# tl32rodan/DCVC

Measured on AMD Instinct MI355X. Metric: encode+decode fps @1920x1080 per GPU; bpp bit-exact + PSNR Δ<1e-4 dB vs ref, higher is better.
Workload: dtype f32 (convs on split-fp16 f16x3 MFMA, fp32 accumulation); 1 GPU; C3 DCVC-DC RGB 1920x1080 (pad 1920x1088) IP=32 write mode; gop=32, precision=split, q_index=0, stream_part=8, parallelism=sequence-sharded x1, 3 GOP lane(s) per GPU, lanes=3, step=one frame on each of 3 lane(s)

## Files before the change

### dcvc_amd/csrc/hip/sdc.hip

```cpp
#include "common.h"
#include "split.h"

namespace {

constexpr int kNW = 8, kNT = kNW * 64;
constexpr int TH = 8, TW = 16;
constexpr int HW_ = TW + 2, NPH = (TH + 2) * HW_;
constexpr int HR = 192;

struct DP {
  const float *x;
  int H, W, xcs, xco;
  float *y;
  int ycs, yco;
  const uint16_t *w;
  int wbytes;
  const float *b1, *wdw, *bdw, *b2, *ba;
  float slope;
  int tiles_x, ntiles;
  int *ovf;
};

template <int CIN, int COUT, bool ADAPT>
struct DG {
  static constexpr int KCI = (CIN + 31) / 32;
  static constexpr int NTI = (CIN + 15) / 16, NTO = (COUT + 15) / 16;
  static constexpr int CI16 = NTI * 16, CO16 = NTO * 16;
  static constexpr int W1 = KCI * CI16 * 32, W2 = KCI * CO16 * 32, WA = ADAPT ? KCI * CO16 * 32 : 0;
  static constexpr int NWH = 2 * (W1 + W2 + WA);
  static constexpr int XI = KCI * HR * 32;
  static constexpr int DI = KCI * TH * TW * 32;
  static constexpr size_t OX = 0, OD = OX + (size_t)2 * XI * 2, OW = OD + (size_t)2 * DI * 2;
  static constexpr size_t OC = OW + (size_t)NWH * 2;
  static constexpr int NC = CIN * 11 + 2 * COUT;
  static constexpr size_t LDS = OC + (size_t)NC * 4;
  static constexpr int QP = CIN / 8;
  static constexpr int PP = (NPH * QP + kNT - 1) / kNT;
};

__device__ __forceinline__ float lrelu(float v, float s) { return fmaxf(v, v * s); }

template <int CIN, int COUT, bool ADAPT>
__global__ void __launch_bounds__(kNT) sdc_kernel(DP p) {
  SplitRange rg(p.ovf);
  typedef DG<CIN, COUT, ADAPT> G_;
  constexpr int KCI = G_::KCI, NTI = G_::NTI, NTO = G_::NTO, CO16 = G_::CO16, CI16 = G_::CI16;
  constexpr int XI = G_::XI, DI = G_::DI, QP = G_::QP, PP = G_::PP;
  extern __shared__ __align__(16) unsigned char smem[];
  uint16_t *Xh = reinterpret_cast<uint16_t *>(smem + G_::OX), *Xl = Xh + XI;
  uint16_t *Dh = reinterpret_cast<uint16_t *>(smem + G_::OD), *Dl = Dh + DI;
  uint16_t *W1h = reinterpret_cast<uint16_t *>(smem + G_::OW), *W1l = W1h + G_::W1;
  uint16_t *W2h = W1l + G_::W1, *W2l = W2h + G_::W2;
  uint16_t *WAh = W2l + G_::W2, *WAl = WAh + G_::WA;
  float *Lb1 = reinterpret_cast<float *>(smem + G_::OC), *Lbdw = Lb1 + CIN, *Lwdw = Lbdw + CIN;
  float *Lb2 = Lwdw + 9 * CIN, *Lba = Lb2 + COUT;
  auto t1p = [&](int r, int c) -> float * {
    return reinterpret_cast<float *>((c & 16) ? Xl : Xh) + (((c >> 5) * HR + r) * 16 + (c & 15));
  };

  const int tid = threadIdx.x;
  const int wave = tid >> 6, lane = tid & 63;
  const int col = lane & 15, hi = lane >> 4;
  const int G = gridDim.x;
  int g = blockIdx.x;
  if ((G & 7) == 0) g = (g & 7) * (G >> 3) + (g >> 3);
  if (g >= p.ntiles) return;

  {
    const __amdgpu_buffer_rsrc_t wr =
        __builtin_amdgcn_make_buffer_rsrc(const_cast<uint16_t *>(p.w), (short)0, p.wbytes, 0x00020000);
    constexpr int ND = G_::NWH * 2 / 1024;
    for (int i = wave; i < ND; i += kNW)
      __builtin_amdgcn_raw_ptr_buffer_load_lds(wr, (__attribute__((address_space(3))) void *)(W1h + i * 512), 16,
                                               i * 1024 + lane * 16, 0, 0, 0);
    for (int i = tid; i < G_::NC; i += kNT) {
      float v;
      if (i < CIN) v = p.b1[i];
      else if (i < 2 * CIN) v = p.bdw[i - CIN];
      else if (i < 11 * CIN) v = p.wdw[i - 2 * CIN];
      else if (i < 11 * CIN + COUT) v = p.b2[i - 11 * CIN];
      else v = ADAPT ? p.ba[i - 11 * CIN - COUT] : 0.f;
      Lb1[i] = v;
    }
  }

  const __amdgpu_buffer_rsrc_t xr = __builtin_amdgcn_make_buffer_rsrc(
      const_cast<float *>(p.x), (short)0,
      (int)((int64_t)p.H * p.W * p.xcs * 4 < 0x7fff0000 ? (int64_t)p.H * p.W * p.xcs * 4 : 0x7fff0000), 0x00020000);
  int pyx[PP], prel[PP], pofs[PP];
#pragma unroll
  for (int u = 0; u < PP; ++u) {
    const int it = tid + u * kNT;
    pyx[u] = -1;
    prel[u] = 0;
    pofs[u] = 0;
    if (it < NPH * QP) {
      const int pix = it / QP, q = it - pix * QP;
      const int hy = pix / HW_, hx = pix - hy * HW_;
      pyx[u] = (hy << 8) | hx;
      prel[u] = ((hy - 1) * p.W + (hx - 1)) * p.xcs + p.xco + q * 8;
      pofs[u] = swz((q >> 2) * HR + pix, q & 3);
    }
  }
  float pf[PP][8];
  auto prefetch = [&](int t) {
    const int oy0 = (t / p.tiles_x) * TH, ox0 = (t % p.tiles_x) * TW;
    const int base = oy0 * p.W + ox0;
#pragma unroll
    for (int u = 0; u < PP; ++u) {
      const int gy = oy0 - 1 + (pyx[u] >> 8), gx = ox0 - 1 + (pyx[u] & 255);
      const bool in = pyx[u] >= 0 && (unsigned)gy < (unsigned)p.H && (unsigned)gx < (unsigned)p.W;
      const int o = in ? (base * p.xcs + prel[u]) * 4 : 0x7fffffe0;
      const f32x4 a = __builtin_bit_cast(f32x4, __builtin_amdgcn_raw_buffer_load_b128(xr, o, 0, 0));
      const f32x4 b = __builtin_bit_cast(f32x4, __builtin_amdgcn_raw_buffer_load_b128(xr, o + 16, 0, 0));
#pragma unroll
      for (int j = 0; j < 4; ++j) {
        pf[u][j] = a[j];
        pf[u][4 + j] = b[j];
      }
    }
  };
  prefetch(g);

  auto zero_pad = [&]() {
    if constexpr (CIN % 32 != 0) {
      constexpr int PADQ = KCI * 4 - QP;
      for (int it = tid; it < HR * PADQ; it += kNT) {
        const int row = it / PADQ, q = QP + it % PADQ;
        const int o = swz((q >> 2) * HR + row, q & 3);
        *reinterpret_cast<u32x4_t *>(Xh + o) = u32x4_t{0u, 0u, 0u, 0u};
        *reinterpret_cast<u32x4_t *>(Xl + o) = u32x4_t{0u, 0u, 0u, 0u};
      }
    }
  };

  wait_vm_lgkm();
  for (int t = g; t < p.ntiles; t += G) {
    const int oy0 = (t / p.tiles_x) * TH, ox0 = (t % p.tiles_x) * TW;
    raw_barrier();
#pragma unroll
    for (int u = 0; u < PP; ++u) {
      u32x4_t h, l;
      rg.add8(pf[u]);
      split8(pf[u], h, l);
      if (pyx[u] >= 0) {
        *reinterpret_cast<u32x4_t *>(Xh + pofs[u]) = h;
        *reinterpret_cast<u32x4_t *>(Xl + pofs[u]) = l;
      }
    }
    zero_pad();
    wait_lgkm();
    raw_barrier();
    if (t + G < p.ntiles) prefetch(t + G);

    f32x4 idn[NTO];
    if constexpr (ADAPT) {
      f32x4 am[NTO], ac[NTO];
#pragma unroll
      for (int j = 0; j < NTO; ++j) {
        am[j] = f32x4{0.f, 0.f, 0.f, 0.f};
        ac[j] = f32x4{0.f, 0.f, 0.f, 0.f};
      }
      const int hr = (wave + 1) * HW_ + 1 + col;
#pragma unroll
      for (int kc = 0; kc < KCI; ++kc) {
        const int ob = swz(kc * HR + hr, hi);
        const f16x8 bh = *reinterpret_cast<const f16x8 *>(Xh + ob), bl = *reinterpret_cast<const f16x8 *>(Xl + ob);
#pragma unroll
        for (int j = 0; j < NTO; ++j) {
          const int oa = swz(kc * CO16 + j * 16 + col, hi);
          const f16x8 ah = *reinterpret_cast<const f16x8 *>(WAh + oa), al = *reinterpret_cast<const f16x8 *>(WAl + oa);
          am[j] = __builtin_amdgcn_mfma_f32_16x16x32_f16(ah, bh, am[j], 0, 0, 0);
          ac[j] = __builtin_amdgcn_mfma_f32_16x16x32_f16(ah, bl, ac[j], 0, 0, 0);
          ac[j] = __builtin_amdgcn_mfma_f32_16x16x32_f16(al, bh, ac[j], 0, 0, 0);
        }
      }
#pragma unroll
      for (int j = 0; j < NTO; ++j) {
        const int n = j * 16 + hi * 4;
#pragma unroll
        for (int e = 0; e < 4; ++e) idn[j][e] = (am[j][e] + ac[j][e] * kLoInv) + Lba[n + e < COUT ? n + e : 0];
      }
      wait_lgkm();
      raw_barrier();
    }

    for (int ht = wave; ht < HR / 16; ht += kNW) {
      f32x4 tm[NTI], tc[NTI];
#pragma unroll
      for (int j = 0; j < NTI; ++j) {
        tm[j] = f32x4{0.f, 0.f, 0.f, 0.f};
        tc[j] = f32x4{0.f, 0.f, 0.f, 0.f};
      }
      const int r = ht * 16 + col;
#pragma unroll
      for (int kc = 0; kc < KCI; ++kc) {
        const int ob = swz(kc * HR + r, hi);
        const f16x8 bh = *reinterpret_cast<const f16x8 *>(Xh + ob), bl = *reinterpret_cast<const f16x8 *>(Xl + ob);
#pragma unroll
        for (int j = 0; j < NTI; ++j) {
          const int oa = swz(kc * CI16 + j * 16 + col, hi);
          const f16x8 ah = *reinterpret_cast<const f16x8 *>(W1h + oa), al = *reinterpret_cast<const f16x8 *>(W1l + oa);
          tm[j] = __builtin_amdgcn_mfma_f32_16x16x32_f16(ah, bh, tm[j], 0, 0, 0);
          tc[j] = __builtin_amdgcn_mfma_f32_16x16x32_f16(ah, bl, tc[j], 0, 0, 0);
          tc[j] = __builtin_amdgcn_mfma_f32_16x16x32_f16(al, bh, tc[j], 0, 0, 0);
        }
      }
      const int hy = r / HW_, hx = r - hy * HW_;
      const int gy = oy0 - 1 + hy, gx = ox0 - 1 + hx;
      const bool inside = r < NPH && (unsigned)gy < (unsigned)p.H && (unsigned)gx < (unsigned)p.W;
      wave_lds_sync();
#pragma unroll
      for (int j = 0; j < NTI; ++j) {
        const int n = j * 16 + hi * 4;
        if (n >= CIN) continue;
        f32x4 v;
#pragma unroll
        for (int e = 0; e < 4; ++e) v[e] = inside ? lrelu((tm[j][e] + tc[j][e] * kLoInv) + Lb1[n + e], p.slope) : 0.f;
        *reinterpret_cast<f32x4 *>(t1p(r, n)) = v;
      }
    }
    wait_lgkm();
    raw_barrier();

    {
      constexpr int CG = CIN / 4;
      constexpr int R = kNT / (CG * TW) >= 4 ? 4 : kNT / (CG * TW) >= 2 ? 2 : 1;
      constexpr int RR = TH / R;
      static_assert(CG * TW * R <= kNT && TH % R == 0, "P2 tasks");
      if (tid < CG * TW * R) {
        const int cg = tid % CG, rest = tid / CG;
        const int ix = rest % TW, y0 = (rest / TW) * RR;
        const int c = cg * 4;
        f32x4 wv[9];
#pragma unroll
        for (int k = 0; k < 9; ++k) wv[k] = *reinterpret_cast<const f32x4 *>(Lwdw + k * CIN + c);
        const float4 bd = *reinterpret_cast<const float4 *>(Lbdw + c);
        f32x4 win[3][3];
#pragma unroll
        for (int r = 0; r < 2; ++r)
#pragma unroll
          for (int dx = 0; dx < 3; ++dx)
            win[r][dx] = *reinterpret_cast<const f32x4 *>(t1p((y0 + r) * HW_ + ix + dx, c));
#pragma unroll
        for (int i = 0; i < RR; ++i) {
#pragma unroll
          for (int dx = 0; dx < 3; ++dx)
            win[(i + 2) % 3][dx] = *reinterpret_cast<const f32x4 *>(t1p((y0 + i + 2) * HW_ + ix + dx, c));
          f32x4 a = f32x4{0.f, 0.f, 0.f, 0.f};
#pragma unroll
          for (int dy = 0; dy < 3; ++dy)
#pragma unroll
            for (int dx = 0; dx < 3; ++dx)
#pragma unroll
              for (int e = 0; e < 4; ++e) a[e] = __builtin_fmaf(wv[dy * 3 + dx][e], win[(i + dy) % 3][dx][e], a[e]);
          float v[4];
          v[0] = a[0] + bd.x;
          v[1] = a[1] + bd.y;
          v[2] = a[2] + bd.z;
          v[3] = a[3] + bd.w;
          rg.add4(v);
          const auto h01 = __builtin_amdgcn_cvt_pkrtz(v[0], v[1]);
          const auto h23 = __builtin_amdgcn_cvt_pkrtz(v[2], v[3]);
          const uint32_t l01 = pk(split_lo(v[0], (float)h01[0]), split_lo(v[1], (float)h01[1]));
          const uint32_t l23 = pk(split_lo(v[2], (float)h23[0]), split_lo(v[3], (float)h23[1]));
          const int px = (y0 + i) * TW + ix;
          const int o = swz((c >> 5) * (TH * TW) + px, (c & 31) >> 3) + (c & 7);
          typedef unsigned int u32x2_t __attribute__((ext_vector_type(2)));
          *reinterpret_cast<u32x2_t *>(Dh + o) = u32x2_t{__builtin_bit_cast(uint32_t, h01), __builtin_bit_cast(uint32_t, h23)};
          *reinterpret_cast<u32x2_t *>(Dl + o) = u32x2_t{l01, l23};
        }
      }
      if constexpr (CIN % 32 != 0) {
        constexpr int PADQ = KCI * 4 - CIN / 8;
        for (int it = tid; it < TH * TW * PADQ; it += kNT) {
          const int px = it / PADQ, q = CIN / 8 + it % PADQ;
          const int o = swz((q >> 2) * (TH * TW) + px, q & 3);
          *reinterpret_cast<u32x4_t *>(Dh + o) = u32x4_t{0u, 0u, 0u, 0u};
          *reinterpret_cast<u32x4_t *>(Dl + o) = u32x4_t{0u, 0u, 0u, 0u};
        }
      }
    }
    wait_lgkm();
    raw_barrier();

    {
      f32x4 cm[NTO], cc[NTO];
#pragma unroll
      for (int j = 0; j < NTO; ++j) {
        cm[j] = f32x4{0.f, 0.f, 0.f, 0.f};
        cc[j] = f32x4{0.f, 0.f, 0.f, 0.f};
      }
#pragma unroll
      for (int kc = 0; kc < KCI; ++kc) {
        const int ob = swz(kc * (TH * TW) + wave * TW + col, hi);
        const f16x8 bh = *reinterpret_cast<const f16x8 *>(Dh + ob), bl = *reinterpret_cast<const f16x8 *>(Dl + ob);
#pragma unroll
        for (int j = 0; j < NTO; ++j) {
          const int oa = swz(kc * CO16 + j * 16 + col, hi);
          const f16x8 ah = *reinterpret_cast<const f16x8 *>(W2h + oa), al = *reinterpret_cast<const f16x8 *>(W2l + oa);
          cm[j] = __builtin_amdgcn_mfma_f32_16x16x32_f16(ah, bh, cm[j], 0, 0, 0);
          cc[j] = __builtin_amdgcn_mfma_f32_16x16x32_f16(ah, bl, cc[j], 0, 0, 0);
          cc[j] = __builtin_amdgcn_mfma_f32_16x16x32_f16(al, bh, cc[j], 0, 0, 0);
        }
      }
      const int gy = oy0 + wave, gx = ox0 + col;
      if (gy < p.H && gx < p.W) {
        const int64_t pix = (int64_t)gy * p.W + gx;
#pragma unroll
        for (int j = 0; j < NTO; ++j) {
          const int n = j * 16 + hi * 4;
          if (n >= COUT) continue;
          f32x4 id;
          if constexpr (ADAPT) id = idn[j];
          else id = *reinterpret_cast<const f32x4 *>(p.x + pix * p.xcs + p.xco + n);
          f32x4 v;
#pragma unroll
          for (int e = 0; e < 4; ++e) v[e] = ((cm[j][e] + cc[j][e] * kLoInv) + Lb2[n + e]) + id[e];
          *reinterpret_cast<f32x4 *>(p.y + pix * p.ycs + p.yco + n) = v;
        }
      }
    }
  }
  wait_vm_lgkm();
}

int g_cus = 0;

template <int CIN, int COUT, bool ADAPT>
int run(DP p, hipStream_t st) {
  typedef DG<CIN, COUT, ADAPT> G_;
  static_assert(G_::LDS <= 160 * 1024, "LDS");
  static_assert(G_::NWH * 2 % 1024 == 0, "weight images in whole 1-KiB pieces");
  p.tiles_x = (p.W + TW - 1) / TW;
  const int64_t nt = (int64_t)p.tiles_x * ((p.H + TH - 1) / TH);
  if (nt <= 0) return DCVC_HIP_OK;
  p.ntiles = (int)nt;
  if (g_cus <= 0) {
    int dev = 0;
    hipDeviceProp_t prop;
    if (hipGetDevice(&dev) != hipSuccess || hipGetDeviceProperties(&prop, dev) != hipSuccess) return DCVC_HIP_ELAUNCH;
    g_cus = prop.multiProcessorCount;
  }
  int G = g_cus;
  if (G > p.ntiles) G = p.ntiles;
  auto kern = sdc_kernel<CIN, COUT, ADAPT>;
  dcvc_note_kernel("sdc_kernel<%d, %d, %s>@%lld", CIN, COUT, bname(ADAPT), (long long)G * kNT);
  dcvc_ensure_lds(reinterpret_cast<const void *>(kern), (int)G_::LDS);
  hipLaunchKernelGGL(kern, dim3((unsigned)G), dim3(kNT), G_::LDS, st, p);
  DCVC_LAUNCH_CHECK();
  return DCVC_HIP_OK;
}

bool supported(int cin, int cout, bool adapt) {
  return (cin == 64 && cout == 48 && adapt) || (cin == 48 && cout == 32 && adapt) ||
         (cin == 64 && cout == 64 && !adapt) || (cin == 32 && cout == 64 && adapt) ||
         (cin == 48 && cout == 48 && !adapt) || (cin == 32 && cout == 32 && !adapt);
}

}

extern "C" int64_t dcvc_dc_pack_weights(const float *w1, const float *w2, const float *wa, int cin, int cout,
                                        void *out) {
  if (!w1 || !w2 || cin <= 0 || cout <= 0) return DCVC_HIP_EINVAL;
  if (out && (!host_split_range_ok(w1, (int64_t)cin * cin) || !host_split_range_ok(w2, (int64_t)cout * cin) ||
              (wa && !host_split_range_ok(wa, (int64_t)cout * cin))))
    return DCVC_HIP_EINVAL;
  const int kci = (cin + 31) / 32, ci16 = (cin + 15) / 16 * 16, co16 = (cout + 15) / 16 * 16;
  const int64_t n1 = (int64_t)kci * ci16 * 32, n2 = (int64_t)kci * co16 * 32, na = wa ? n2 : 0;
  const int64_t total = 2 * (n1 + n2 + na);
  if (!out) return total;
  uint16_t *o = reinterpret_cast<uint16_t *>(out);
  auto at = [](int row, int k) {
    const int x = (0x1320 >> (((row >> 2) & 3) << 2)) & 3;
    return (int64_t)row * 32 + ((((k >> 3) ^ x) & 3) << 3) + (k & 7);
  };
  auto put = [&](uint16_t *img, int64_t n, const float *w, int rows, int rows16) {
    for (int kc = 0; kc < kci; ++kc)
      for (int r = 0; r < rows16; ++r)
        for (int k = 0; k < 32; ++k) {
          const int ch = kc * 32 + k;
          const float v = (r < rows && ch < cin) ? w[(int64_t)r * cin + ch] : 0.f;
          const int64_t q = at(kc * rows16 + r, k);
          host_split(v, img[q], img[n + q]);
        }
  };
  put(o, n1, w1, cin, ci16);
  put(o + 2 * n1, n2, w2, cout, co16);
  if (wa) put(o + 2 * n1 + 2 * n2, na, wa, cout, co16);
  return total;
}

extern "C" int dcvc_depth_conv_split(const dcvc_dc_args *a, void *stream) {
  if (!a || !a->x.ptr || !a->y.ptr || !a->w || !a->b1 || !a->wdw || !a->bdw || !a->b2) return DCVC_HIP_EINVAL;
  if (a->x.dtype != DCVC_F32 || a->y.dtype != DCVC_F32 || a->x.C != a->cin || a->y.C != a->cout ||
      a->x.H != a->y.H || a->x.W != a->y.W)
    return DCVC_HIP_EINVAL;
  const bool adapt = a->adaptor != 0;
  if (!supported(a->cin, a->cout, adapt) || (adapt && !a->ba)) return DCVC_HIP_EUNSUPPORTED;
  if (!(a->slope >= 0.f && a->slope <= 1.f)) return DCVC_HIP_EUNSUPPORTED;
  if (a->x.cstride % 4 || a->x.coff % 4 || a->y.cstride % 4 || a->y.coff % 4 || ((uintptr_t)a->x.ptr & 15) ||
      ((uintptr_t)a->y.ptr & 15))
    return DCVC_HIP_EUNSUPPORTED;
  if ((int64_t)a->x.H * a->x.W * a->x.cstride * 4 >= 0x7fff0000) return DCVC_HIP_EUNSUPPORTED;
  DP p{};
  p.ovf = dcvc_internal_split_flag();
  p.x = reinterpret_cast<const float *>(a->x.ptr);
  p.H = a->x.H;
  p.W = a->x.W;
  p.xcs = a->x.cstride;
  p.xco = a->x.coff;
  p.y = reinterpret_cast<float *>(a->y.ptr);
  p.ycs = a->y.cstride;
  p.yco = a->y.coff;
  p.w = reinterpret_cast<const uint16_t *>(a->w);
  p.wbytes = (int)(dcvc_dc_pack_weights(reinterpret_cast<const float *>(1), reinterpret_cast<const float *>(1),
                                        adapt ? reinterpret_cast<const float *>(1) : nullptr, a->cin, a->cout,
                                        nullptr) * 2);
  p.b1 = a->b1;
  p.wdw = a->wdw;
  p.bdw = a->bdw;
  p.b2 = a->b2;
  p.ba = a->ba;
  p.slope = a->slope;
  hipStream_t st = reinterpret_cast<hipStream_t>(stream);
  if (a->cin == 64 && a->cout == 48) return run<64, 48, true>(p, st);
  if (a->cin == 48 && a->cout == 32) return run<48, 32, true>(p, st);
  if (a->cin == 32 && a->cout == 64) return run<32, 64, true>(p, st);
  if (a->cin == 64 && a->cout == 64) return run<64, 64, false>(p, st);
  if (a->cin == 48 && a->cout == 48) return run<48, 48, false>(p, st);
  return run<32, 32, false>(p, st);
}
```

### dcvc_amd/layers.py

```python
import torch

from . import hip as K
from .hip import Act, F32, BF16, F16X3, ACT_LRELU, ACT_NONE, IN_LRELU, IN_GATE


FUSE_DCB = True
FUSE_FFN = True
FUSE_DC = True
DW128 = True
SDC_SHAPES = {(64, 48, True), (48, 32, True), (32, 64, True), (64, 64, False), (48, 48, False), (32, 32, False)}


class Precision:
    def __init__(self, feat, feat_compute, latent_compute):
        self.feat = feat
        self.feat_compute = feat_compute
        self.latent = F32
        self.latent_compute = latent_compute

    @staticmethod
    def parity():
        return Precision(F32, F32, F32)

    @staticmethod
    def fast(latent_compute=F32):
        return Precision(BF16, BF16, latent_compute)

    @staticmethod
    def split():
        return Precision(F32, F16X3, F16X3)

    @property
    def name(self):
        if self.feat_compute == F16X3:
            return "split"
        if self.feat == F32:
            return "parity"
        return "fast" if self.latent_compute == F32 else "fast-bf16-tail"


def split_checkpoint(codec, stage):
    if codec.prec.feat_compute == F16X3 and getattr(codec, "_guard_on", False):
        K.split_guard_check(f"{type(codec).__name__}.{stage}")


def parity_twin(codec):
    t = getattr(codec, "_parity_twin", None)
    if t is None:
        kw = dict(codec._init_kw, precision=Precision.parity(), device=codec.dev)
        t = type(codec)(**kw).load_state_dict(codec.sd)
        if codec.entropy_coder is not None:
            t.update(force=True)
        codec._parity_twin = t
    if codec.entropy_coder is not None:
        t.entropy_coder = codec.entropy_coder
    return t


def split_guarded(fn):
    import functools

    @functools.wraps(fn)
    def run(self, *args, **kw):
        if self.prec.feat_compute != F16X3:
            return fn(self, *args, **kw)
        ec = self.entropy_coder
        trace = getattr(ec, "trace", None) if ec is not None else None
        n0 = len(trace) if trace is not None else 0
        K.split_guard_arm(self.dev)
        self._guard_on = True
        try:
            out = fn(self, *args, **kw)
            K.split_guard_check(f"{type(self).__name__}.encode_decode")
            return out
        except K.SplitRangeError as e:
            reason = str(e)
        finally:
            self._guard_on = False
            K.split_guard_disarm()
        if trace is not None:
            del trace[n0:]
        self.fallbacks = getattr(self, "fallbacks", 0) + 1
        out = parity_twin(self).encode_decode(*args, **kw)
        out["precision_fallback"] = "parity"
        out["precision_fallback_reason"] = reason
        return out
    return run


class Ctx:

    def __init__(self, state_dict, device, prec):
        self.sd = state_dict
        self.dev = device
        self.prec = prec
        self.used = set()

    def has(self, name):
        return name + ".weight" in self.sd

    def take(self, key):
        if key not in self.sd:
            raise KeyError(f"missing key in state_dict: {key}")
        self.used.add(key)
        return self.sd[key]

    def check_strict(self, extra_used=()):
        unused = set(self.sd) - self.used - set(extra_used)
        if unused:
            raise RuntimeError(f"unexpected key(s) in state_dict: {sorted(unused)[:8]}")

    def conv(self, name, stride=1, latent=False, compute=None, cin_pad=None, out_perm=None, in_perm=None):
        if compute is None:
            compute = self.prec.latent_compute if latent else self.prec.feat_compute
        b = self.take(name + ".bias") if name + ".bias" in self.sd else None
        w = self.take(name + ".weight")
        if in_perm is not None:
            w = w.detach().float()[:, torch.as_tensor(in_perm, dtype=torch.long)]
        if cin_pad is not None and cin_pad > w.shape[1]:
            w = torch.nn.functional.pad(w.detach().float(), (0, 0, 0, 0, 0, cin_pad - w.shape[1]))
        if out_perm is not None:
            perm = torch.as_tensor(out_perm, dtype=torch.long)
            w = w.detach().float()[perm]
            if b is not None:
                b = b.detach().float()[perm]
        return K.ConvW(w, b, stride, compute, self.dev)

    def dw(self, name):
        w = self.take(name + ".weight").detach().float().cpu()
        C = w.shape[0]
        w9c = w.reshape(C, 9).t().contiguous().to(self.dev)
        b = self.take(name + ".bias").detach().float().contiguous().to(self.dev)
        return w9c, b

    def dtype(self, latent):
        return self.prec.latent if latent else self.prec.feat

    def fit(self, x, compute):
        if compute != BF16 and x.dtype != F32:
            return cast(x, F32)
        return x


def cast(x, dtype):
    if x.dtype == dtype:
        return x
    y = K.empty(x.H, x.W, x.C, dtype, x.buf.device)
    return K.copy(x, y)


class DepthConvBlock:

    def __init__(self, ctx, p, gated=False, latent=False, slope_dc=0.01, slope_ffn=0.1):
        self.ctx, self.latent, self.gated = ctx, latent, gated
        self.slope_dc, self.slope_ffn = slope_dc, slope_ffn
        d = p + ".block.0"
        f = p + ".block.1"
        self.conv1 = ctx.conv(d + ".conv1.0", latent=latent)
        self.dw = ctx.dw(d + ".depth_conv")
        self.conv2 = ctx.conv(d + ".conv2", latent=latent)
        self.adaptor = ctx.conv(d + ".adaptor", latent=latent) if ctx.has(d + ".adaptor") else None
        if gated:
            self.ffn1 = ctx.conv(f + ".conv", latent=latent)
            self.ffn2 = ctx.conv(f + ".conv_out", latent=latent)
        else:
            self.ffn1 = ctx.conv(f + ".conv.0", latent=latent)
            self.ffn2 = ctx.conv(f + ".conv.2", latent=latent)
        self.cout = self.ffn2.cout
        self.dcw = None
        sd = ctx.sd
        if (FUSE_DC and self.conv1.compute == F16X3 and not latent and
                (self.conv1.cin, self.conv2.cout, self.adaptor is not None) in SDC_SHAPES):
            self.dcw = K.DcW(sd[d + ".conv1.0.weight"], sd[d + ".conv1.0.bias"], self.dw[0], self.dw[1],
                             sd[d + ".conv2.weight"], sd[d + ".conv2.bias"],
                             sd[d + ".adaptor.weight"] if self.adaptor is not None else None,
                             sd[d + ".adaptor.bias"] if self.adaptor is not None else None, ctx.dev)
        self.dwc = None
        if (FUSE_DC and self.conv1.compute == F16X3 and self.adaptor is None and self.conv1.cin == self.conv2.cout
                and ((latent and self.conv2.cin in (192, 384)) or (DW128 and not latent and self.conv2.cin == 128))):
            self.dwc = K.DwcW(self.dw[0], self.dw[1], sd[d + ".conv2.weight"], sd[d + ".conv2.bias"], ctx.dev)
        self.ffn = None
        if (FUSE_FFN and not gated and self.ffn2.compute == F16X3 and self.cout in (32, 48, 64, 128, 192, 384)
                and self.ffn1.cout % (64 if self.cout != 128 else 32) == 0):
            sd = ctx.sd
            self.ffn = K.FfnW(sd[f + ".conv.0.weight"], sd[f + ".conv.0.bias"], sd[f + ".conv.2.weight"],
                              sd[f + ".conv.2.bias"], ctx.dev)

    def __call__(self, x, y=None, scale=None):
        ctx = self.ctx
        dt = ctx.dtype(self.latent)
        if (FUSE_DCB and not self.latent and x.dtype == BF16 and dt == BF16
                and self.conv1.compute == BF16 and self.cout <= 128 and x.C <= 128):
            out = y if y is not None else K.empty(x.H, x.W, self.cout, BF16, x.buf.device)
            if K.depthconv_block(self, x, out, scale) is not None:
                return out
        x = ctx.fit(x, self.conv1.compute)
        dc = None
        if self.dcw is not None:
            dc = K.depth_conv_split(self.dcw, x, slope=self.slope_dc)
        if dc is not None:
            pass
        elif self.adaptor is not None:
            idn = K.conv(self.adaptor, x, out_dtype=dt)
        else:
            idn = cast(x, dt)
        if dc is None:
            t = K.conv(self.conv1, x, out_dtype=dt, act=ACT_LRELU, slope=self.slope_dc)
            if self.dwc is not None:
                dc = K.dw_conv2_split(self.dwc, t, idn)
            if dc is None:
                t = K.dwconv3x3(t, *self.dw)
                dc = K.conv(self.conv2, t, res=idn)
        if self.gated:
            h = K.conv(self.ffn1, dc)
            return K.conv(self.ffn2, h, y, in_op=IN_GATE, in_slope=self.slope_ffn, res=dc, scale=scale)
        if self.ffn is not None:
            out = K.conv_ffn(self.ffn, dc, y, scale=scale, slope=self.slope_ffn)
            if out is not None:
                return out
        hid = BF16 if self.ffn2.compute == BF16 else dt
        h = K.conv(self.ffn1, dc, out_dtype=hid, act=ACT_LRELU, slope=self.slope_ffn)
        return K.conv(self.ffn2, h, y, out_dtype=dc.dtype, act=ACT_LRELU, slope=self.slope_ffn, res=dc,
                      scale=scale)


class ResidualBlockWithStride:

    def __init__(self, ctx, p, latent=False):
        self.ctx, self.latent = ctx, latent
        self.conv1 = ctx.conv(p + ".conv1", 2, latent)
        self.conv2 = ctx.conv(p + ".conv2", 1, latent)
        self.down = ctx.conv(p + ".downsample", 2, latent)

    def __call__(self, x, y=None, scale=None):
        dt = self.ctx.dtype(self.latent)
        x = self.ctx.fit(x, self.conv1.compute)
        t = K.conv(self.conv1, x, out_dtype=dt, act=ACT_LRELU, slope=0.01)
        idn = K.conv(self.down, x, out_dtype=dt)
        return K.conv(self.conv2, t, y, act=ACT_LRELU, slope=0.1, res=idn, scale=scale)


class ResidualBlockUpsample:

    def __init__(self, ctx, p, latent=False):
        self.ctx, self.latent = ctx, latent
        self.sub = ctx.conv(p + ".subpel_conv.0", 1, latent)
        self.conv = ctx.conv(p + ".conv", 1, latent)
        self.up = ctx.conv(p + ".upsample.0", 1, latent)

    def __call__(self, x, y=None, scale=None):
        dt = self.ctx.dtype(self.latent)
        x = self.ctx.fit(x, self.sub.compute)
        t = K.conv(self.sub, x, out_dtype=dt, shuffle=True, act=ACT_LRELU, slope=0.01)
        idn = K.conv(self.up, x, out_dtype=dt, shuffle=True)
        return K.conv(self.conv, t, y, act=ACT_LRELU, slope=0.1, res=idn, scale=scale)


class ResBlock:

    def __init__(self, ctx, p, slope=0.01, end_with_relu=False, latent=False):
        self.ctx, self.latent = ctx, latent
        self.slope, self.end = slope, end_with_relu
        self.conv1 = ctx.conv(p + ".conv1", 1, latent)
        self.conv2 = ctx.conv(p + ".conv2", 1, latent)

    def __call__(self, x, y=None, res2=None, scale=None):
        t = K.conv(self.conv1, x, in_op=IN_LRELU, in_slope=self.slope, act=ACT_LRELU, slope=self.slope)
        return K.conv(self.conv2, t, y, act=ACT_LRELU if self.end else ACT_NONE, slope=self.slope,
                      res=x, res2=res2, scale=scale)


class UNet:

    def __init__(self, ctx, p, gated=False):
        self.ctx = ctx
        B = lambda n: DepthConvBlock(ctx, f"{p}.{n}", gated=gated)
        self.conv1, self.conv2, self.conv3 = B("conv1"), B("conv2"), B("conv3")
        self.refine = [B(f"context_refine.{i}") for i in range(4)]
        self.up3 = ctx.conv(p + ".up3.0")
        self.up_conv3 = B("up_conv3")
        self.up2 = ctx.conv(p + ".up2.0")
        self.up_conv2 = B("up_conv2")

    def __call__(self, x, y=None):
        dt = self.ctx.prec.feat
        H, W = x.H, x.W
        c1 = self.conv1.cout
        c2 = self.conv2.cout
        cat2 = K.empty(H, W, c1 + self.up2.cout // 4, dt, x.buf.device)
        x1 = self.conv1(x, cat2.ch(0, c1))
        x2p = K.pool2x2(x1, True)
        cat3 = K.empty(H // 2, W // 2, c2 + self.up3.cout // 4, dt, x.buf.device)
        x2 = self.conv2(x2p, cat3.ch(0, c2))
        x3 = self.conv3(K.pool2x2(x2, True))
        for b in self.refine:
            x3 = b(x3)
        K.conv(self.up3, x3, cat3.ch(c2, self.up3.cout // 4), shuffle=True)
        d3 = self.up_conv3(cat3)
        K.conv(self.up2, d3, cat2.ch(c1, self.up2.cout // 4), shuffle=True)
        return self.up_conv2(cat2, y)


class SpyNet:

    def __init__(self, ctx, p, grids):
        self.ctx, self.grids = ctx, grids
        self.levels = [[ctx.conv(f"{p}.moduleBasic.{lv}.conv{i}") for i in range(1, 6)] for lv in range(4)]

    def __call__(self, im1, im2):
        dev = im1.buf.device
        p1, p2 = [im1], [im2]
        for _ in range(3):
            p1.append(K.pool2x2(p1[-1], False))
            p2.append(K.pool2x2(p2[-1], False))
        flow = K.zeros(p2[3].H // 2, p2[3].W // 2, 2, F32, dev)
        cdt = self.ctx.prec.feat_compute
        in_dt = F32 if cdt == F32 else self.ctx.prec.feat
        for lv in range(4):
            k = 3 - lv
            H, W = p1[k].H, p1[k].W
            cat = K.empty(H, W, 8, F32, dev)
            flow_up = K.resize2x(flow, True, 2.0, y=cat.ch(6, 2))
            K.copy(p1[k], cat.ch(0, 3))
            K.flow_warp(p2[k], flow_up, self.grids(H, W), y=cat.ch(3, 3))
            convs = self.levels[lv]
            t = cast(cat, in_dt)
            for c in convs[:4]:
                t = K.conv(c, t, out_dtype=in_dt, act=ACT_LRELU, slope=0.0)
            flow = K.conv(convs[4], t, out_dtype=F32, res=cast(flow_up, F32) if flow_up.dtype != F32 else flow_up)
        return flow


def hyper_enc(ctx, p, reduce_enc_layer):
    if reduce_enc_layer:
        convs = [(ctx.conv(p + ".0", 1, True), True), (ctx.conv(p + ".2", 2, True), True),
                 (ctx.conv(p + ".4", 2, True), False)]
    else:
        convs = [(ctx.conv(p + ".0", 1, True), True), (ctx.conv(p + ".2", 1, True), True),
                 (ctx.conv(p + ".4", 2, True), True), (ctx.conv(p + ".6", 1, True), True),
                 (ctx.conv(p + ".8", 2, True), False)]

    def run(x):
        for c, relu in convs:
            x = K.conv(c, ctx.fit(x, c.compute), out_dtype=F32, act=ACT_LRELU if relu else K.ACT_ROUND,
                       slope=0.01)
        return x
    return run


def hyper_dec(ctx, p):
    c0, c4, c8 = (ctx.conv(f"{p}.{i}", 1, True) for i in (0, 4, 8))
    c2, c6 = (ctx.conv(f"{p}.{i}.0", 1, True) for i in (2, 6))

    def run(x, y=None):
        x = K.conv(c0, x, act=ACT_LRELU, slope=0.01)
        x = K.conv(c2, x, shuffle=True, act=ACT_LRELU, slope=0.01)
        x = K.conv(c4, x, act=ACT_LRELU, slope=0.01)
        x = K.conv(c6, x, shuffle=True, act=ACT_LRELU, slope=0.01)
        return K.conv(c8, x, y)
    return run


class Grids:

    def __init__(self, device):
        self.dev = device
        self.cache = {}

    def __call__(self, H, W):
        key = (H, W)
        if key not in self.cache:
            gx = torch.linspace(-1.0, 1.0, W, dtype=torch.float32).to(self.dev)
            gy = torch.linspace(-1.0, 1.0, H, dtype=torch.float32).to(self.dev)
            self.cache[key] = (gx, gy)
        return self.cache[key]
```

Baseline: 30.28 frames/s.

## Add 4-row-tile fused depthwise-conv block kernel for 128-channel shapes

Adds a second variant of the fused 1x1 -> depthwise 3x3 -> 1x1 (+adapter/residual) kernel. It uses 4-row tiles and streams weights into LDS in phases when they do not fit, and it is enabled for the 128/128, 64->128 and 128->64 shapes that previously fell back to separate kernels. The aim is to remove intermediate global-memory round trips and extra launches for the wide layers. In exchange, smaller tiles mean more halo recomputation, and weight re-streaming per tile adds DMA and barrier overhead.

After: 30.65 frames/s (median of 6 runs). No clear change (+1.2%).

```diff
diff --git a/dcvc_amd/csrc/hip/sdc.hip b/dcvc_amd/csrc/hip/sdc.hip
--- a/dcvc_amd/csrc/hip/sdc.hip
+++ b/dcvc_amd/csrc/hip/sdc.hip
@@ -352,10 +352,360 @@
   return DCVC_HIP_OK;
 }
 
+constexpr int TH4 = 4;
+constexpr int NPH4 = (TH4 + 2) * HW_;
+constexpr int HR4 = 112;
+
+__device__ __forceinline__ uint32_t lds_addr(const void *p) {
+#ifdef __HIP_DEVICE_COMPILE__
+  return (uint32_t)(uintptr_t)(const __attribute__((address_space(3))) void *)p;
+#else
+  return (uint32_t)(uintptr_t)p;
+#endif
+}
+__device__ __forceinline__ f16x8 lds_frag(uint32_t a, int bytes) {
+#ifdef __HIP_DEVICE_COMPILE__
+  return *(const __attribute__((address_space(3))) f16x8 *)(a + (uint32_t)bytes);
+#else
+  (void)a, (void)bytes;
+  return f16x8{};
+#endif
+}
+
+template <int CIN, int COUT, bool ADAPT>
+struct DG4 {
+  static_assert(CIN % 32 == 0 && COUT % 32 == 0, "whole 32-channel chunks, an even number of 16-channel blocks");
+  static constexpr int KCI = CIN / 32, NTI = CIN / 16, NTO = COUT / 16;
+  static constexpr int W1 = KCI * CIN * 32, W2 = KCI * COUT * 32, WA = ADAPT ? KCI * COUT * 32 : 0;
+  static constexpr int XI = KCI * HR4 * 32, DI = KCI * TH4 * TW * 32;
+  static constexpr int NC = CIN * 11 + 2 * COUT;
+  static constexpr size_t OX = 0, OD = OX + (size_t)2 * XI * 2, OW = OD + (size_t)2 * DI * 2;
+  static constexpr int BA = 4 * W1, BB = 4 * (W2 + WA);
+  static constexpr bool STREAM = OW + BA + BB + (size_t)NC * 4 > 160 * 1024;
+  static constexpr size_t OWB = STREAM ? OW : OW + BA;
+  static constexpr size_t OC = STREAM ? OW + (BA > BB ? BA : BB) : OW + BA + BB;
+  static constexpr size_t LDS = OC + (size_t)NC * 4;
+  static constexpr int QP = CIN / 8;
+  static constexpr int PP = (NPH4 * QP + kNT - 1) / kNT;
+};
+
+template <int CIN, int COUT, bool ADAPT, int TILE_H>
+__global__ void __launch_bounds__(kNT) sdc_kernel(DP p) {
+  static_assert(TILE_H == TH4, "the 4-row tile kernel");
+  SplitRange rg(p.ovf);
+  typedef DG4<CIN, COUT, ADAPT> G_;
+  constexpr int KCI = G_::KCI, NTI = G_::NTI, NTO = G_::NTO, NJ = NTO / 2;
+  constexpr int XI = G_::XI, DI = G_::DI, QP = G_::QP, PP = G_::PP;
+  constexpr bool STREAM = G_::STREAM;
+  extern __shared__ __align__(16) unsigned char smem[];
+  uint16_t *Xh = reinterpret_cast<uint16_t *>(smem + G_::OX), *Xl = Xh + XI;
+  uint16_t *Dh = reinterpret_cast<uint16_t *>(smem + G_::OD), *Dl = Dh + DI;
+  uint16_t *W1h = reinterpret_cast<uint16_t *>(smem + G_::OW), *W2h = reinterpret_cast<uint16_t *>(smem + G_::OWB);
+  float *Lb1 = reinterpret_cast<float *>(smem + G_::OC), *Lbdw = Lb1 + CIN, *Lwdw = Lbdw + CIN;
+  float *Lb2 = Lwdw + 9 * CIN, *Lba = Lb2 + COUT;
+  auto t1p = [&](int r, int c) -> float * {
+    return reinterpret_cast<float *>((c & 16) ? Xl : Xh) + (((c >> 5) * HR4 + r) * 16 + (c & 15));
+  };
+
+  const int tid = threadIdx.x;
+  const int wave = tid >> 6, lane = tid & 63;
+  const int col = lane & 15, hi = lane >> 4;
+  const int prow = wave & 3, jb = (wave >> 2) * NJ;
+  static_assert(G_::BA <= 65536 && G_::BB <= 65536 && 2 * XI * 2 <= 65536, "ds_read offsets are 16 bits");
+  const uint32_t aw1_ = lds_addr(W1h + swz(col, hi));
+  const uint32_t aw2_ = lds_addr(W2h + swz(col, hi));
+  const uint32_t ai_ = lds_addr(Xh + swz((prow + 1) * HW_ + 1 + col, hi));
+  const uint32_t ad_ = lds_addr(Dh + swz(prow * TW + col, hi));
+  const int G = gridDim.x;
+  int g = blockIdx.x;
+  if ((G & 7) == 0) g = (g & 7) * (G >> 3) + (g >> 3);
+  if (g >= p.ntiles) return;
+
+  const __amdgpu_buffer_rsrc_t wr =
+      __builtin_amdgcn_make_buffer_rsrc(const_cast<uint16_t *>(p.w), (short)0, p.wbytes, 0x00020000);
+  auto dma = [&](uint16_t *dst, int src, int bytes) {
+    for (int i = wave; i < bytes / 1024; i += kNW)
+      __builtin_amdgcn_raw_ptr_buffer_load_lds(wr, (__attribute__((address_space(3))) void *)(dst + i * 512), 16,
+                                               src + i * 1024 + lane * 16, 0, 0, 0);
+  };
+  if constexpr (!STREAM) dma(W1h, 0, G_::BA);
+  dma(W2h, G_::BA, G_::BB);
+  for (int i = tid; i < G_::NC; i += kNT) {
+    float v;
+    if (i < CIN) v = p.b1[i];
+    else if (i < 2 * CIN) v = p.bdw[i - CIN];
+    else if (i < 11 * CIN) v = p.wdw[i - 2 * CIN];
+    else if (i < 11 * CIN + COUT) v = p.b2[i - 11 * CIN];
+    else v = ADAPT ? p.ba[i - 11 * CIN - COUT] : 0.f;
+    Lb1[i] = v;
+  }
+
+  const __amdgpu_buffer_rsrc_t xr = __builtin_amdgcn_make_buffer_rsrc(
+      const_cast<float *>(p.x), (short)0,
+      (int)((int64_t)p.H * p.W * p.xcs * 4 < 0x7fff0000 ? (int64_t)p.H * p.W * p.xcs * 4 : 0x7fff0000), 0x00020000);
+  int pyx[PP], prel[PP], pofs[PP];
+#pragma unroll
+  for (int u = 0; u < PP; ++u) {
+    const int it = tid + u * kNT;
+    pyx[u] = -1;
+    prel[u] = 0;
+    pofs[u] = 0;
+    if (it < NPH4 * QP) {
+      static_assert(NPH4 % 4 == 0 && QP % 4 == 0, "publish lane layout");
+      const int grp = it >> 4;
+      const int pix = (grp / (QP / 4)) * 4 + ((it >> 2) & 3), q = (it & 3) | ((grp % (QP / 4)) << 2);
+      const int hy = pix / HW_, hx = pix - hy * HW_;
+      pyx[u] = (hy << 8) | hx;
+      prel[u] = ((hy - 1) * p.W + (hx - 1)) * p.xcs + p.xco + q * 8;
+      pofs[u] = swz((q >> 2) * HR4 + pix, q & 3);
+    }
+  }
+  float pf[PP][8];
+  auto prefetch = [&](int t) {
+    const int oy0 = (t / p.tiles_x) * TH4, ox0 = (t % p.tiles_x) * TW;
+    const int base = oy0 * p.W + ox0;
+#pragma unroll
+    for (int u = 0; u < PP; ++u) {
+      const int gy = oy0 - 1 + (pyx[u] >> 8), gx = ox0 - 1 + (pyx[u] & 255);
+      const bool in = pyx[u] >= 0 && (unsigned)gy < (unsigned)p.H && (unsigned)gx < (unsigned)p.W;
+      const int o = in ? (base * p.xcs + prel[u]) * 4 : 0x7fffffe0;
+      const f32x4 a = __builtin_bit_cast(f32x4, __builtin_amdgcn_raw_buffer_load_b128(xr, o, 0, 0));
+      const f32x4 b = __builtin_bit_cast(f32x4, __builtin_amdgcn_raw_buffer_load_b128(xr, o + 16, 0, 0));
+#pragma unroll
+      for (int j = 0; j < 4; ++j) {
+        pf[u][j] = a[j];
+        pf[u][4 + j] = b[j];
+      }
+    }
+  };
+  prefetch(g);
+
+  wait_vm_lgkm();
+  for (int t = g; t < p.ntiles; t += G) {
+    const int oy0 = (t / p.tiles_x) * TH4, ox0 = (t % p.tiles_x) * TW;
+    uint32_t aw1 = aw1_, aw2 = aw2_, ai = ai_, ad = ad_;
+    opaque_v(aw1);
+    opaque_v(aw2);
+    opaque_v(ai);
+    opaque_v(ad);
+    raw_barrier();
+    if constexpr (STREAM && !ADAPT) dma(W1h, 0, G_::BA);
+#pragma unroll
+    for (int u = 0; u < PP; ++u) {
+      u32x4_t h, l;
+      rg.add8(pf[u]);
+      split8(pf[u], h, l);
+      if (pyx[u] >= 0) {
+        *reinterpret_cast<u32x4_t *>(Xh + pofs[u]) = h;
+        *reinterpret_cast<u32x4_t *>(Xl + pofs[u]) = l;
+      }
+    }
+    if constexpr (STREAM && !ADAPT) wait_vm_lgkm();
+    else wait_lgkm();
+    raw_barrier();
+
+    f32x4 idn[NJ];
+    if constexpr (ADAPT) {
+      f32x4 am[NJ], ac[NJ];
+#pragma unroll
+      for (int j = 0; j < NJ; ++j) {
+        am[j] = f32x4{0.f, 0.f, 0.f, 0.f};
+        ac[j] = f32x4{0.f, 0.f, 0.f, 0.f};
+      }
+#pragma unroll
+      for (int kc = 0; kc < KCI; ++kc) {
+        const f16x8 bh = lds_frag(ai, kc * HR4 * 64), bl = lds_frag(ai, kc * HR4 * 64 + XI * 2);
+#pragma unroll
+        for (int j = 0; j < NJ; ++j) {
+          const int oa = 4 * G_::W2 + (kc * COUT + (jb + j) * 16) * 64;
+          const f16x8 ah = lds_frag(aw2, oa), al = lds_frag(aw2, oa + G_::WA * 2);
+          am[j] = __builtin_amdgcn_mfma_f32_16x16x32_f16(ah, bh, am[j], 0, 0, 0);
+          ac[j] = __builtin_amdgcn_mfma_f32_16x16x32_f16(ah, bl, ac[j], 0, 0, 0);
+          ac[j] = __builtin_amdgcn_mfma_f32_16x16x32_f16(al, bh, ac[j], 0, 0, 0);
+        }
+      }
+#pragma unroll
+      for (int j = 0; j < NJ; ++j) {
+        const int n = (jb + j) * 16 + hi * 4;
+#pragma unroll
+        for (int e = 0; e < 4; ++e) idn[j][e] = (am[j][e] + ac[j][e] * kLoInv) + Lba[n + e];
+      }
+      wait_lgkm();
+      raw_barrier();
+      if constexpr (STREAM) {
+        dma(W1h, 0, G_::BA);
+        wait_vm_lgkm();
+        raw_barrier();
+      }
+    }
+    if (t + G < p.ntiles) prefetch(t + G);
+
+    for (int ht = wave; ht < HR4 / 16; ht += kNW) {
+      f32x4 tm[NTI], tc[NTI];
+#pragma unroll
+      for (int j = 0; j < NTI; ++j) {
+        tm[j] = f32x4{0.f, 0.f, 0.f, 0.f};
+        tc[j] = f32x4{0.f, 0.f, 0.f, 0.f};
+      }
+      const int r = ht * 16 + col;
+      uint32_t ax = lds_addr(Xh + swz(r, hi));
+      opaque_v(ax);
+#pragma unroll
+      for (int kc = 0; kc < KCI; ++kc) {
+        const f16x8 bh = lds_frag(ax, kc * HR4 * 64), bl = lds_frag(ax, kc * HR4 * 64 + XI * 2);
+#pragma unroll
+        for (int j = 0; j < NTI; ++j) {
+          const int oa = (kc * CIN + j * 16) * 64;
+          const f16x8 ah = lds_frag(aw1, oa), al = lds_frag(aw1, oa + G_::W1 * 2);
+          tm[j] = __builtin_amdgcn_mfma_f32_16x16x32_f16(ah, bh, tm[j], 0, 0, 0);
+          tc[j] = __builtin_amdgcn_mfma_f32_16x16x32_f16(ah, bl, tc[j], 0, 0, 0);
+          tc[j] = __builtin_amdgcn_mfma_f32_16x16x32_f16(al, bh, tc[j], 0, 0, 0);
+        }
+      }
+      const int hy = r / HW_, hx = r - hy * HW_;
+      const int gy = oy0 - 1 + hy, gx = ox0 - 1 + hx;
+      const bool inside = r < NPH4 && (unsigned)gy < (unsigned)p.H && (unsigned)gx < (unsigned)p.W;
+      wave_lds_sync();
+#pragma unroll
+      for (int j = 0; j < NTI; ++j) {
+        const int n = j * 16 + hi * 4;
+        f32x4 v;
+#pragma unroll
+        for (int e = 0; e < 4; ++e) v[e] = inside ? lrelu((tm[j][e] + tc[j][e] * kLoInv) + Lb1[n + e], p.slope) : 0.f;
+        *reinterpret_cast<f32x4 *>(t1p(r, n)) = v;
+      }
+    }
+    wait_lgkm();
+    raw_barrier();
+    if constexpr (STREAM) dma(W2h, G_::BA, G_::BB);
+
+    {
+      constexpr int CG = CIN / 4;
+      constexpr int R = kNT / (CG * TW) >= 2 ? 2 : 1;
+      constexpr int RR = TH4 / R;
+      static_assert(CG * TW * R <= kNT && TH4 % R == 0, "P2 tasks");
+      static_assert(CG % 4 == 0 && TW == 16, "P2 lane layout");
+      if (tid < CG * TW * R) {
+        const int rest = tid >> 6;
+        const int cg = (tid & 3) | ((rest % (CG / 4)) << 2);
+        const int ix = (tid >> 2) & 15, y0 = (rest / (CG / 4)) * RR;
+        const int c = cg * 4;
+        f32x4 wv[9];
+#pragma unroll
+        for (int k = 0; k < 9; ++k) wv[k] = *reinterpret_cast<const f32x4 *>(Lwdw + k * CIN + c);
+        const float4 bd = *reinterpret_cast<const float4 *>(Lbdw + c);
+        f32x4 win[3][3];
+#pragma unroll
+        for (int r = 0; r < 2; ++r)
+#pragma unroll
+          for (int dx = 0; dx < 3; ++dx)
+            win[r][dx] = *reinterpret_cast<const f32x4 *>(t1p((y0 + r) * HW_ + ix + dx, c));
+#pragma unroll
+        for (int i = 0; i < RR; ++i) {
+#pragma unroll
+          for (int dx = 0; dx < 3; ++dx)
+            win[(i + 2) % 3][dx] = *reinterpret_cast<const f32x4 *>(t1p((y0 + i + 2) * HW_ + ix + dx, c));
+          f32x4 a = f32x4{0.f, 0.f, 0.f, 0.f};
+#pragma unroll
+          for (int dy = 0; dy < 3; ++dy)
+#pragma unroll
+            for (int dx = 0; dx < 3; ++dx)
+#pragma unroll
+              for (int e = 0; e < 4; ++e) a[e] = __builtin_fmaf(wv[dy * 3 + dx][e], win[(i + dy) % 3][dx][e], a[e]);
+          float v[4];
+          v[0] = a[0] + bd.x;
+          v[1] = a[1] + bd.y;
+          v[2] = a[2] + bd.z;
+          v[3] = a[3] + bd.w;
+          rg.add4(v);
+          const auto h01 = __builtin_amdgcn_cvt_pkrtz(v[0], v[1]);
+          const auto h23 = __builtin_amdgcn_cvt_pkrtz(v[2], v[3]);
+          const uint32_t l01 = pk(split_lo(v[0], (float)h01[0]), split_lo(v[1], (float)h01[1]));
+          const uint32_t l23 = pk(split_lo(v[2], (float)h23[0]), split_lo(v[3], (float)h23[1]));
+          const int px = (y0 + i) * TW + ix;
+          const int o = swz((c >> 5) * (TH4 * TW) + px, (c & 31) >> 3) + (c & 7);
+          typedef unsigned int u32x2_t __attribute__((ext_vector_type(2)));
+          *reinterpret_cast<u32x2_t *>(Dh + o) = u32x2_t{__builtin_bit_cast(uint32_t, h01), __builtin_bit_cast(uint32_t, h23)};
+          *reinterpret_cast<u32x2_t *>(Dl + o) = u32x2_t{l01, l23};
+        }
+      }
+    }
+    if constexpr (STREAM) wait_vm_lgkm();
+    else wait_lgkm();
+    raw_barrier();
+
+    {
+      f32x4 cm[NJ], cc[NJ];
+#pragma unroll
+      for (int j = 0; j < NJ; ++j) {
+        cm[j] = f32x4{0.f, 0.f, 0.f, 0.f};
+        cc[j] = f32x4{0.f, 0.f, 0.f, 0.f};
+      }
+#pragma unroll
+      for (int kc = 0; kc < KCI; ++kc) {
+        const f16x8 bh = lds_frag(ad, kc * (TH4 * TW) * 64), bl = lds_frag(ad, kc * (TH4 * TW) * 64 + DI * 2);
+#pragma unroll
+        for (int j = 0; j < NJ; ++j) {
+          const int oa = (kc * COUT + (jb + j) * 16) * 64;
+          const f16x8 ah = lds_frag(aw2, oa), al = lds_frag(aw2, oa + G_::W2 * 2);
+          cm[j] = __builtin_amdgcn_mfma_f32_16x16x32_f16(ah, bh, cm[j], 0, 0, 0);
+          cc[j] = __builtin_amdgcn_mfma_f32_16x16x32_f16(ah, bl, cc[j], 0, 0, 0);
+          cc[j] = __builtin_amdgcn_mfma_f32_16x16x32_f16(al, bh, cc[j], 0, 0, 0);
+        }
+      }
+      const int gy = oy0 + prow, gx = ox0 + col;
+      if (gy < p.H && gx < p.W) {
+        const int64_t pix = (int64_t)gy * p.W + gx;
+#pragma unroll
+        for (int j = 0; j < NJ; ++j) {
+          const int n = (jb + j) * 16 + hi * 4;
+          f32x4 id;
+          if constexpr (ADAPT) id = idn[j];
+          else id = *reinterpret_cast<const f32x4 *>(p.x + pix * p.xcs + p.xco + n);
+          f32x4 v;
+#pragma unroll
+          for (int e = 0; e < 4; ++e) v[e] = ((cm[j][e] + cc[j][e] * kLoInv) + Lb2[n + e]) + id[e];
+          *reinterpret_cast<f32x4 *>(p.y + pix * p.ycs + p.yco + n) = v;
+        }
+      }
+    }
+  }
+  wait_vm_lgkm();
+}
+
+template <int CIN, int COUT, bool ADAPT>
+int run4(DP p, hipStream_t st) {
+  typedef DG4<CIN, COUT, ADAPT> G_;
+  static_assert(G_::LDS <= 160 * 1024, "LDS");
+  static_assert(G_::BA % 1024 == 0 && G_::BB % 1024 == 0, "weight images in whole 1-KiB pieces");
+  static_assert(G_::NTO % 2 == 0, "P1a / P3 split the output-channel blocks over two wave groups");
+  p.tiles_x = (p.W + TW - 1) / TW;
+  const int64_t nt = (int64_t)p.tiles_x * ((p.H + TH4 - 1) / TH4);
+  if (nt <= 0) return DCVC_HIP_OK;
+  if (nt > 0x7fffffff) return DCVC_HIP_EUNSUPPORTED;
+  p.ntiles = (int)nt;
+  if (g_cus <= 0) {
+    int dev = 0;
+    hipDeviceProp_t prop;
+    if (hipGetDevice(&dev) != hipSuccess || hipGetDeviceProperties(&prop, dev) != hipSuccess) return DCVC_HIP_ELAUNCH;
+    g_cus = prop.multiProcessorCount;
+  }
+  int G = g_cus;
+  if (G > p.ntiles) G = p.ntiles;
+  auto kern = sdc_kernel<CIN, COUT, ADAPT, TH4>;
+  dcvc_note_kernel("sdc_kernel<%d, %d, %s, %d>@%lld", CIN, COUT, bname(ADAPT), TH4, (long long)G * kNT);
+  dcvc_ensure_lds(reinterpret_cast<const void *>(kern), (int)G_::LDS);
+  hipLaunchKernelGGL(kern, dim3((unsigned)G), dim3(kNT), G_::LDS, st, p);
+  DCVC_LAUNCH_CHECK();
+  return DCVC_HIP_OK;
+}
+
 bool supported(int cin, int cout, bool adapt) {
   return (cin == 64 && cout == 48 && adapt) || (cin == 48 && cout == 32 && adapt) ||
          (cin == 64 && cout == 64 && !adapt) || (cin == 32 && cout == 64 && adapt) ||
-         (cin == 48 && cout == 48 && !adapt) || (cin == 32 && cout == 32 && !adapt);
+         (cin == 48 && cout == 48 && !adapt) || (cin == 32 && cout == 32 && !adapt) ||
+         (cin == 128 && cout == 128 && !adapt) || (cin == 64 && cout == 128 && adapt) ||
+         (cin == 128 && cout == 64 && adapt);
 }
 
 }
@@ -424,6 +774,9 @@
   p.ba = a->ba;
   p.slope = a->slope;
   hipStream_t st = reinterpret_cast<hipStream_t>(stream);
+  if (a->cin == 128 && a->cout == 128) return run4<128, 128, false>(p, st);
+  if (a->cin == 64 && a->cout == 128) return run4<64, 128, true>(p, st);
+  if (a->cin == 128 && a->cout == 64) return run4<128, 64, true>(p, st);
   if (a->cin == 64 && a->cout == 48) return run<64, 48, true>(p, st);
   if (a->cin == 48 && a->cout == 32) return run<48, 32, true>(p, st);
   if (a->cin == 32 && a->cout == 64) return run<32, 64, true>(p, st);
diff --git a/dcvc_amd/layers.py b/dcvc_amd/layers.py
--- a/dcvc_amd/layers.py
+++ b/dcvc_amd/layers.py
@@ -8,7 +8,8 @@
 FUSE_FFN = True
 FUSE_DC = True
 DW128 = True
-SDC_SHAPES = {(64, 48, True), (48, 32, True), (32, 64, True), (64, 64, False), (48, 48, False), (32, 32, False)}
+SDC_SHAPES = {(64, 48, True), (48, 32, True), (32, 64, True), (64, 64, False), (48, 48, False), (32, 32, False),
+              (128, 128, False), (64, 128, True), (128, 64, True)}
 
 
 class Precision:
```
